# mcbuehler/DeepSEE

Measured on AMD Instinct MI355X. Metric: train-step images/sec (G+D fwd+bwd), 8x 32->256 bs=8, higher is better.
Workload: dtype fp32

## Files before the change

### deepsee_amd/csrc/elementwise.hip

```cpp
#include "dsee_common.h"
#include "dsee_rng.h"

namespace {

inline int egrid(long n) { return (int)min(8192L, (n + 255) / 256); }

__global__ __launch_bounds__(256) void up_noise_fwd_kernel(const float* __restrict__ x, const float* __restrict__ eps,
                                                           const float* __restrict__ nw, float* __restrict__ y, int N,
                                                           int H, int W, int C, int ups) {
  const long total4 = (long)N * H * W * C / 4;
  const int C4 = C / 4, h0 = H >> ups, w0 = W >> ups;
  for (long i = blockIdx.x * (long)blockDim.x + threadIdx.x; i < total4; i += (long)gridDim.x * blockDim.x) {
    const dsee_nhwq p = dsee_split_nhwq((unsigned)i, C4, W, H);
    const int q = p.q;
    f32x4 v = *reinterpret_cast<const f32x4*>(x + (((size_t)p.n * h0 + (p.h >> ups)) * w0 + (p.w >> ups)) * C + q * 4);
    if (eps) v += *reinterpret_cast<const f32x4*>(nw + q * 4) * *reinterpret_cast<const f32x4*>(eps + i * 4);
    *reinterpret_cast<f32x4*>(y + i * 4) = v;
  }
}

__global__ __launch_bounds__(256) void sumpool_kernel(const float* __restrict__ dy, float* __restrict__ dx, int N, int H,
                                                      int W, int C, int ups, float* __restrict__ amax = nullptr) {
  float vmax = 0.f;
  const int h0 = H >> ups, w0 = W >> ups, C4 = C / 4, f = 1 << ups;
// ... 368 lines not shown
                                                                uint64_t offset, const uint64_t* __restrict__ epoch) {
  if (epoch) offset += *epoch;
  __shared__ f32x4 red[256];
  const int tpp = C / 4, ppb = 256 / tpp > 0 ? 256 / tpp : 1;
  const int q = threadIdx.x % tpp, s = threadIdx.x / tpp;
  const bool active = threadIdx.x < ppb * tpp;
  const long p0 = (long)blockIdx.x * chunk_px, p1 = min(M, p0 + chunk_px);
  f32x4 acc = {0.f, 0.f, 0.f, 0.f};
  if (active)
    for (long p = p0 + s; p < p1; p += ppb)
      acc += *reinterpret_cast<const f32x4*>(a + p * C + q * 4) * philox_normal4(seed, offset + (uint64_t)(p * tpp + q));
  if (active) red[s * tpp + q] = acc;
  __syncthreads();
  if (active && s == 0) {
    f32x4 v = red[q];
    for (int j = 1; j < ppb; ++j) v += red[j * tpp + q];
    *reinterpret_cast<f32x4*>(part + (size_t)blockIdx.x * C + q * 4) = v;
  }
}

__global__ __launch_bounds__(256) void sumpool_dot_rng_kernel(const float* __restrict__ dy, float* __restrict__ dx, int N, int H,
                                                              int W, int C, int ups, float* __restrict__ amax,
                                                              float* __restrict__ part, uint64_t seed, uint64_t offset,
                                                              const uint64_t* __restrict__ epoch) {
  if (epoch) offset += *epoch;
  __shared__ f32x4 red[256];
  float vmax = 0.f;
  f32x4 acc = {0.f, 0.f, 0.f, 0.f};
  const int h0 = H >> ups, w0 = W >> ups, C4 = C / 4, f = 1 << ups;
  const long total4 = (long)N * h0 * w0 * C4;
  for (long i = blockIdx.x * (long)blockDim.x + threadIdx.x; i < total4; i += (long)gridDim.x * blockDim.x) {
    const dsee_nhwq p = dsee_split_nhwq((unsigned)i, C4, w0, h0);
    f32x4 v = {0.f, 0.f, 0.f, 0.f};
    for (int a = 0; a < f; ++a)
      for (int b = 0; b < f; ++b) {
        const size_t px = ((size_t)p.n * H + p.h * f + a) * W + p.w * f + b;
        const f32x4 d = *reinterpret_cast<const f32x4*>(dy + px * C + p.q * 4);
        v += d;
        acc += d * philox_normal4(seed, offset + (uint64_t)(px * C4 + p.q));
      }
    *reinterpret_cast<f32x4*>(dx + i * 4) = v;
    vmax = fmaxf(vmax, dsee_absmax4(v));
  }
  if (amax) dsee_block_atomic_absmax(amax, vmax);
  red[threadIdx.x] = acc;
  __syncthreads();
  if ((int)threadIdx.x < C4) {
    f32x4 s = red[threadIdx.x];
    for (int k = threadIdx.x + C4; k < 256; k += C4) s += red[k];
    *reinterpret_cast<f32x4*>(part + (size_t)blockIdx.x * C + threadIdx.x * 4) = s;
  }
}

}

extern "C" {

int dsee_upsample_noise_rng_fwd(const float* x, const float* noise_w, float* y, int N, int H, int W, int C, int ups,
                                uint64_t seed, uint64_t offset, hipStream_t st) {
  DSEE_CHECK_ARG(x && y && noise_w && C % 4 == 0);
  DSEE_CHECK_ARG((long)N * H * W * C / 4 < (1L << 32));
  up_noise_rng_fwd_kernel<false><<<egrid((long)N * H * W * C / 4), 256, 0, st>>>(x, noise_w, y, N, H, W, C, ups, seed, offset,
                                                                                 dsee_rng_epoch(), nullptr);
  DSEE_LAUNCH_CHECK();
  return DSEE_OK;
}

int dsee_upsample_noise_rng_fwd_stats(const float* x, const float* noise_w, float* y, int N, int H, int W, int C, int ups,
                                      uint64_t seed, uint64_t offset, float* stats_part, hipStream_t st) {
  DSEE_CHECK_ARG(x && y && noise_w && stats_part && C % 4 == 0 && C / 4 <= 256 && 256 % (C / 4) == 0);
  DSEE_CHECK_ARG((long)N * H * W * C / 4 < (1L << 32));
  const long items = (long)N * H * W * C / 4;
  const int grid = (int)min((long)DSEE_STATS_ROWS_MAX, (items + 255) / 256);
  up_noise_rng_fwd_kernel<true><<<grid, 256, 0, st>>>(x, noise_w, y, N, H, W, C, ups, seed, offset, dsee_rng_epoch(),
                                                      stats_part);
  DSEE_LAUNCH_CHECK();
  return DSEE_OK;
}

int dsee_channel_dot_rng(const float* a, float* out, long M, int C, float* workspace, uint64_t seed, uint64_t offset,
                         hipStream_t st) {
  DSEE_CHECK_ARG(a && out && workspace && C % 4 == 0 && C <= 1024);
  long cp = (M + 1023) / 1024;
  if (cp < 64) cp = 64;
  const int parts = (int)((M + cp - 1) / cp);
  chdot_rng_partial_kernel<<<parts, 256, 0, st>>>(a, workspace, M, C, (int)cp, seed, offset, dsee_rng_epoch());
  DSEE_LAUNCH_CHECK();
  chdot_finalize_kernel<<<C / 4, 256, 0, st>>>(workspace, parts, C, out);
  DSEE_LAUNCH_CHECK();
  return DSEE_OK;
}

int dsee_upsample_noise_fwd(const float* x, const float* eps, const float* noise_w, float* y, int N, int H, int W, int C,
                            int ups, hipStream_t st) {
  DSEE_CHECK_ARG(x && y && C % 4 == 0 && (eps == nullptr || noise_w != nullptr));
  DSEE_CHECK_ARG((long)N * H * W * C / 4 < (1L << 32));
  up_noise_fwd_kernel<<<egrid((long)N * H * W * C / 4), 256, 0, st>>>(x, eps, noise_w, y, N, H, W, C, ups);
  DSEE_LAUNCH_CHECK();
  return DSEE_OK;
}

int dsee_sumpool(const float* dy, float* dx, int N, int H, int W, int C, int ups, hipStream_t st) {
  DSEE_CHECK_ARG(dy && dx && C % 4 == 0 && ups >= 1);
  DSEE_CHECK_ARG((long)N * H * W * C / 4 < (1L << 32));
  sumpool_kernel<<<egrid((long)N * (H >> ups) * (W >> ups) * C / 4), 256, 0, st>>>(dy, dx, N, H, W, C, ups);
  DSEE_LAUNCH_CHECK();
  return DSEE_OK;
}

int dsee_sumpool_amax(const float* dy, float* dx, int N, int H, int W, int C, int ups, float* amax_dx, hipStream_t st) {
  DSEE_CHECK_ARG(dy && dx && amax_dx && C % 4 == 0 && ups >= 1);
  DSEE_CHECK_ARG((long)N * H * W * C / 4 < (1L << 32));
  sumpool_kernel<<<egrid((long)N * (H >> ups) * (W >> ups) * C / 4), 256, 0, st>>>(dy, dx, N, H, W, C, ups, amax_dx);
  DSEE_LAUNCH_CHECK();
  return DSEE_OK;
}

size_t dsee_sumpool_dot_rng_workspace(int N, int H, int W, int C, int ups) {
  return (size_t)egrid((long)N * (H >> ups) * (W >> ups) * C / 4) * C * sizeof(float);
}
int dsee_sumpool_dot_rng(const float* dy, float* dx, int N, int H, int W, int C, int ups, float* amax_dx, float* dnoise_w,
                         float* workspace, uint64_t seed, uint64_t offset, hipStream_t st) {
  DSEE_CHECK_ARG(dy && dx && dnoise_w && workspace && C % 4 == 0 && ups >= 1 && 256 % (C / 4) == 0);
  DSEE_CHECK_ARG((long)N * H * W * C / 4 < (1L << 32));
  const int grid = egrid((long)N * (H >> ups) * (W >> ups) * C / 4);
  sumpool_dot_rng_kernel<<<grid, 256, 0, st>>>(dy, dx, N, H, W, C, ups, amax_dx, workspace, seed, offset, dsee_rng_epoch());
  DSEE_LAUNCH_CHECK();
  chdot_finalize_kernel<<<C / 4, 256, 0, st>>>(workspace, grid, C, dnoise_w);
  DSEE_LAUNCH_CHECK();
  return DSEE_OK;
}

size_t dsee_channel_dot_workspace(long M, int C) {
  long cp = (M + 1023) / 1024;
  if (cp < 64) cp = 64;
  return (size_t)((M + cp - 1) / cp) * C * sizeof(float);
}

int dsee_channel_dot(const float* a, const float* b, float* out, long M, int C, float* workspace, hipStream_t st) {
  DSEE_CHECK_ARG(a && out && workspace && C % 4 == 0 && C <= 1024);
  long cp = (M + 1023) / 1024;
  if (cp < 64) cp = 64;
  const int parts = (int)((M + cp - 1) / cp);
  chdot_partial_kernel<<<parts, 256, 0, st>>>(a, b, workspace, M, C, (int)cp);
  DSEE_LAUNCH_CHECK();
  chdot_finalize_kernel<<<C / 4, 256, 0, st>>>(workspace, parts, C, out);
  DSEE_LAUNCH_CHECK();
  return DSEE_OK;
}

int dsee_act_fwd(const float* x, float* y, long n, int act, float slope, hipStream_t st) {
  DSEE_CHECK_ARG(x && y && n % 4 == 0);
  act_fwd_kernel<<<egrid(n / 4), 256, 0, st>>>(x, y, n / 4, act, slope);
  DSEE_LAUNCH_CHECK();
  return DSEE_OK;
}

int dsee_act_bwd(const float* dy, const float* y, float* dx, long n, int act, float slope, hipStream_t st) {
  DSEE_CHECK_ARG(dy && y && dx && n % 4 == 0);
  act_bwd_kernel<<<egrid(n / 4), 256, 0, st>>>(dy, y, dx, n / 4, act, slope);
  DSEE_LAUNCH_CHECK();
  return DSEE_OK;
}

int dsee_act_bwd_amax(const float* dy, const float* y, float* dx, long n, int act, float slope, float* amax_dx,
                      hipStream_t st) {
  DSEE_CHECK_ARG(dy && y && dx && amax_dx && n % 4 == 0);
  act_bwd_kernel<<<egrid(n / 4), 256, 0, st>>>(dy, y, dx, n / 4, act, slope, amax_dx);
  DSEE_LAUNCH_CHECK();
  return DSEE_OK;
}

int dsee_axpby(const float* a, float alpha, const float* b, float beta, float* y, long n, hipStream_t st) {
  DSEE_CHECK_ARG(a && y && n % 4 == 0);
  axpby_kernel<<<egrid(n / 4), 256, 0, st>>>(a, alpha, b, beta, y, n / 4);
  DSEE_LAUNCH_CHECK();
  return DSEE_OK;
}

int dsee_avgpool3s2_fwd(const float* x, float* y, int N, int H, int W, int C, hipStream_t st) {
  DSEE_CHECK_ARG(x && y && C % 4 == 0);
  const int Ho = (H + 2 - 3) / 2 + 1, Wo = (W + 2 - 3) / 2 + 1;
  avgpool3s2_fwd_kernel<<<egrid((long)N * Ho * Wo * C / 4), 256, 0, st>>>(x, y, N, H, W, Ho, Wo, C);
  DSEE_LAUNCH_CHECK();
  return DSEE_OK;
// ... 97 lines not shown
```

### deepsee_amd/networks.py

```python
import math
import re

import torch
import torch.nn as nn

from . import lib as L
from . import ops

NHIDDEN = ops.NHIDDEN


class Holder(nn.Module):
    """Pure container used to reproduce nn.Sequential-style key paths ('mlp_shared.0.weight')."""


def attach(root, dotted, module):
    parts = dotted.split(".")
    cur = root
    for p in parts[:-1]:
        if not hasattr(cur, p):
            cur.add_module(p, Holder())
        cur = getattr(cur, p)
    cur.add_module(parts[-1], module)
    return module
# ... 306 lines not shown
            actv = ops.SeanInput.apply(sh.weight, sh.bias, None, labels, shift, True, False)
        if self.kind == "spade":
            cat = ops.SeanInput.apply(sh.weight, sh.bias, None, labels, shift, True, False)
            w2, b2 = ops.pack_gamma_beta(self.mlp_gamma.weight, self.mlp_beta.weight, self.mlp_gamma.bias,
                                         self.mlp_beta.bias)
            add_one = 1.0
        elif self.kind == "sean":
            wg, wb = torch.sigmoid(self.alpha_gamma), torch.sigmoid(self.alpha_beta)
            if capped:
                wgam = (1.0 - wg) * self.mlp_gamma.weight + wg * self.mlp_style_gamma.weight
                wbet = (1.0 - wb) * self.mlp_beta.weight + wb * self.mlp_style_beta.weight
                cat = actv
            else:
                cat = ops.SeanInput.apply(sh.weight, sh.bias, style, labels, shift, True, True)
                wgam = torch.cat([(1.0 - wg) * self.mlp_gamma.weight, wg * self.mlp_style_gamma.weight], 1)
                wbet = torch.cat([(1.0 - wb) * self.mlp_beta.weight, wb * self.mlp_style_beta.weight], 1)
            bg = (1.0 - wg) * self.mlp_gamma.bias + wg * self.mlp_style_gamma.bias
            bb = (1.0 - wb) * self.mlp_beta.bias + wb * self.mlp_style_beta.bias
            w2, b2 = ops.pack_gamma_beta(wgam, wbet, bg, bb)
            add_one = 1.0
        else:
            cat = actv if capped else ops.SeanInput.apply(sh.weight, sh.bias, style, labels, shift, False, True)
            w2, b2 = ops.pack_gamma_beta(self.mlp_style_gamma.weight, self.mlp_style_beta.weight,
                                         self.mlp_style_gamma.bias, self.mlp_style_beta.bias)
            add_one = 0.0
        return ops.SpadeNormAct.apply(x, cat, w2, b2, *self._running(), training, add_one, cat_ups,
                                      grad_sink)


class SPADEResnetBlock(nn.Module):

    def __init__(self, c, opt, kind):
        super().__init__()
        self.kind, self.add_noise_cfg = kind, bool(opt.add_noise)
        self.conv_0 = SNConvP(c, c, 3, True)
        self.conv_1 = SNConvP(c, c, 3, True)
        norm = param_free_norm_of(opt.norm_G) if hasattr(opt, "norm_G") else "batch"
        self.norm_0 = SpadeNorm(kind, c, opt.semantic_nc, opt.regional_style_size, opt.max_fm_size, norm)
        self.norm_1 = SpadeNorm(kind, c, opt.semantic_nc, opt.regional_style_size, opt.max_fm_size, norm)
        if self.add_noise_cfg:
            self.noise_in, self.noise_skip, self.noise_middle = VecP(c), VecP(c), VecP(c)

    def forward(self, x, labels, style, noise, tag, ups, training, out_act=L.ACT_NONE, defer_act_bwd=False):
        noisy = self.add_noise_cfg and training
        n, h0, w0, c = x.shape
        shp = (n, h0 << ups, w0 << ups, c)
        res_noise = None
        if noisy:
            x = ops.UpNoise.apply(x, self.noise_in.weight, noise.normal_nhwc(shp, tag + ".noise_in"), ups, training)
            res_noise = (self.noise_skip.weight, noise.normal_nhwc(shp, tag + ".noise_skip"))
        elif ups:
            x = ops.UpNoise.apply(x, None, None, ups)
        sink = ops.GradSink() if (torch.is_grad_enabled() and x.requires_grad) else None
        h = self.norm_0(x, labels, style, training, sink)
        dx = ops.conv2d(h, self.conv_0.weight(training), self.conv_0.bias,
                        noise=(self.noise_middle.weight, noise.normal_nhwc(shp, tag + ".noise_middle")) if noisy else None,
                        stats=training)
        h = self.norm_1(dx, labels, style, training)
        return ops.conv2d(h, self.conv_1.weight(training), self.conv_1.bias, res=x, act=out_act, res_noise=res_noise,
                          res_sink=sink, defer_act_bwd=defer_act_bwd)


class DeepSEESR(nn.Module):

    def __init__(self, opt, plan):
        super().__init__()
        c = 16 * opt.ngf
        self.c = c
        self.initial = ConvP(c, 3, 3)
        self.head_0 = SPADEResnetBlock(c, opt, plan[0][1])
        self.G_middle_0 = SPADEResnetBlock(c, opt, plan[1][1])
        self.G_middle_1 = SPADEResnetBlock(c, opt, plan[2][1])
        self.up_list = nn.ModuleList([SPADEResnetBlock(c, opt, k) for _, k in plan[3:]])
        self.conv_img = ConvP(3, c, 3)
        self._sn = None

    def forward(self, image_lr, labels, style, noise, training):
        blocks = [("head_0", self.head_0, 0), ("G_middle_0", self.G_middle_0, 1), ("G_middle_1", self.G_middle_1, 0)]
        blocks += [("up_list.%d" % i, b, 1) for i, b in enumerate(self.up_list)]
        if self._sn is None:
            self._sn = ops.SNGroup([c for _, b, _ in blocks for c in (b.conv_0, b.conv_1)])
        self._sn.run(training)
        self._sn.wino_weights(torch.is_grad_enabled())
        x = ops.conv2d(image_lr, self.initial.weight, self.initial.bias)
        for i, (tag, blk, ups) in enumerate(blocks):
            last = i == len(blocks) - 1
            defer = last and torch.is_grad_enabled() and x.requires_grad and ops.P().defer_act
            x = blk(x, labels, style, noise, tag, ups, training, L.ACT_LRELU if last else L.ACT_NONE, defer)
        return ops.conv2d(x, self.conv_img.weight, self.conv_img.bias, act=L.ACT_TANH, in_act=L.ACT_LRELU if defer else 0)


class EncBranch(nn.Module):

    def __init__(self, names, strides, ups, nf, cin, norm="instance"):
        super().__init__()
        chans = [(nf, cin), (2 * nf, nf), (4 * nf, 2 * nf), (8 * nf, 4 * nf)]
        self.names, self.strides, self.ups = names, strides, ups
        self.norm_layers = [NormConv(self, nm, co, ci, 3, norm) for nm, (co, ci) in zip(names, chans)]

    def convs(self):
        return [nl.conv(self) for nl in self.norm_layers]

    def forward_main(self, x, training):
        for nl, s, u in zip(self.norm_layers, self.strides, self.ups):
            x = nl.apply(self, x, nl.conv(self).weight(training), L.ACT_LRELU, training, stride=s, pad=1, ups=u)
        return x
# ... 172 lines not shown
```

### deepsee_amd/ops.py

```python
import os
import ctypes as C

import threading

import torch

from . import lib as L
from .plan import KernelPlan, DEFAULT_PLAN, current as P

LRELU_SLOPE = 0.2
BN_EPS = 1e-5
BN_MOMENTUM = 0.1
SN_EPS = 1e-12
NHIDDEN = 128

_scratch = {}

PROFILE = None
PROFILE_BYTES = {}
PROFILE_OPERAND_GB = 0.0


def _variant(geom, modulate=False):
    halo = (geom.korder == 1 and geom.KH == 3 and geom.KW == 3 and geom.mul == 1 and geom.Hi == geom.Ho
# ... 803 lines not shown
            gd = L.geom_dgrad(geom)
            dxl = conv_raw(g, _pack_dgrad(w, geom.Cout, gd.korder), gd, amax_cache=getattr(ctx, "amax_cache", None),
                           exact=ctx.exact)
            if geom.ups:
                dx = torch.empty_like(x)
                L.call("sumpool", dxl, dx, geom.N, gd.Ho, gd.Wo, geom.Cin, geom.ups)
            else:
                dx = dxl
        if dw is not None or thin1:
            pass
        elif ctx.needs_input_grad[1] and ctx.thin:
            ws = scratch(L.lib().dsee_conv3x3_thin_wgrad_workspace(geom.Cin), "wgrad")
            dw = new(co, ci, 3, 3)
            L.call("conv3x3_thin_wgrad", x, g, ws, dw, geom.N, geom.Hi, geom.Wi, geom.Cin, co, ci)
        elif ctx.needs_input_grad[1] and ctx.wino and P().winograd_wgrad:
            dw = _wino_wgrad(x, g, geom.N, geom.Hi, geom.Wi, geom.Cin, geom.Cout, co, ci, vkeep, sums=sums)
        elif ctx.needs_input_grad[1]:
            dw = wgrad_raw(x, g, geom, co, ci, kh, kw, amax_cache=getattr(ctx, "amax_cache", None), exact=ctx.exact)
        if sums is not None and sums.get("dbias") is not None:
            db = sums["dbias"][:co]
        elif ctx.has_bias and ctx.needs_input_grad[2]:
            db = channel_dot(g, None, co).clone()
        if ctx.has_res and ctx.needs_input_grad[3]:
            if ctx.res_sink is not None:
                ctx.res_sink.put(g)
            else:
                dres = g

        def noise_wgrad(eps):
            cn = g.shape[-1]
            mrows = g.numel() // cn
            d = new(cn)
            L.call("channel_dot_rng", g, d, mrows, cn, scratch(L.lib().dsee_channel_dot_workspace(mrows, cn), "chdot"),
                   eps.seed, eps.offset)
            return d

        if sums is not None and "dn0" in sums:
            dnw, drnw = sums["dn0"], sums["dn1"]
        else:
            dnw = noise_wgrad(ctx.noise) if (ctx.noise is not None and ctx.needs_input_grad[8]) else None
            drnw = noise_wgrad(ctx.res_noise) if (ctx.res_noise is not None and ctx.needs_input_grad[10]) else None
        if ctx.in_act and dx is not None and not thin1:
            gx = torch.empty_like(dx)
            tag_amax(gx, amax_slot())
            L.call("act_bwd_amax", dx.contiguous(), x, gx, C.c_long(dx.numel()), ctx.in_act, LRELU_SLOPE, gx.dsee_amax)
            dx = gx
        return dx, dw, db, dres, None, None, None, None, dnw, None, drnw, None, None, None, None, None, None


class GradSink:

    def __init__(self):
        self.g = None

    def put(self, g):
        if self.g is not None:
            raise RuntimeError("GradSink holds a gradient nobody took: the previous backward pass did not reach the "
                               "normalisation that consumes it (partial backward passes are not supported)")
        self.g = g

    def take(self):
        g, self.g = self.g, None
        return g


def _fusable_noise(x, w, stride, pad, ups, eps):
    n, hi, wi, cin_s = x.shape
    return (P().fuse_noise and isinstance(eps, PhiloxNormal) and w.shape[2] == 3 and w.shape[0] > 4
            and _wino_ok(n, hi, wi, cin_s, L.pad4(w.shape[0]), 3, stride, pad, ups))


class ThinGather(torch.autograd.Function):
    @staticmethod
    def forward(ctx, z, bias, co, act, kh=3, kw=3, pad=1):
        n, h, w, ldz = z.shape
        ho, wo = h + 2 * pad - kh + 1, w + 2 * pad - kw + 1
        out = new(n, ho, wo, 4)
        if (kh, kw, pad) == (3, 3, 1):
            L.call("thin_gather_fwd", z, bias, out, n, h, w, ldz, co, act, LRELU_SLOPE)
        else:
            L.call("thin_gather_k_fwd", z, bias, out, n, h, w, ldz, co, kh, kw, pad, act, LRELU_SLOPE)
        ctx.save_for_backward(out)
        ctx.meta = (co, act, ldz, bias is not None, kh, kw, pad, h, w)
        return out

    @staticmethod
    def backward(ctx, dout):
        (out,) = ctx.saved_tensors
        co, act, ldz, has_bias, kh, kw, pad, h, w = ctx.meta
        n = out.shape[0]
        dout = dout.contiguous()
        dz = new(n, h, w, ldz)
        if (kh, kw, pad) == (3, 3, 1):
            L.call("thin_gather_bwd", dout, out, dz, n, h, w, ldz, co, act, LRELU_SLOPE)
        else:
            L.call("thin_gather_k_bwd", dout, out, dz, n, h, w, ldz, co, kh, kw, pad, act, LRELU_SLOPE)
        db = None
        if has_bias and ctx.needs_input_grad[1]:
            g = torch.empty_like(dout)
            L.call("act_bwd", dout, out, g, C.c_long(dout.numel()), act, LRELU_SLOPE)
            db = channel_dot(g, None, co).clone()
        return dz, db, None, None, None, None, None


def _thin_ok(x, w, res, stride, pad, ups, noise, res_noise):
    co, ci, kh, kw = w.shape
# ... 183 lines not shown
            L.call("counter_inc", counter)
        y = torch.empty_like(x)
        ao = amax_slot() if (_direct_split_on() and P().conv_amax_out) else None
        L.call("bn_act_fwd", x, mean, invstd, gamma, beta, y, n, h * w, c, act, LRELU_SLOPE, ao)
        if ao is not None:
            tag_amax(y, ao)
        ctx.act, ctx.emit_amax, ctx.cfg, ctx.training = act, ao is not None, cfg, training
        ctx.save_for_backward(x, y, mean, invstd, gamma)
        return y

    @staticmethod
    def backward(ctx, dy):
        assert ctx.training, "BatchNormAct: backward of an eval-mode forward"
        x, y, mean, invstd, gamma = ctx.saved_tensors
        n, h, w, c = x.shape
        dy = dy.contiguous()
        sums = new(2, c)
        ws = scratch(L.lib().dsee_norm_workspace(n, h * w, c, 1), "norm")
        L.call("bn_act_bwd_reduce", dy, y, x, mean, invstd, n, h * w, c, ctx.act, LRELU_SLOPE, sums, ws)
        count, local, cfg = n * h * w, None, ctx.cfg
        if cfg is not None:
            from . import parallel
            local = sums.clone()
            parallel.allreduce_sums(sums, cfg.world, cfg.group)
            count *= cfg.world
        dgamma = new(c) if ctx.needs_input_grad[1] else None
        dbeta = new(c) if ctx.needs_input_grad[2] else None
        dx = torch.empty_like(x)
        ao = amax_slot() if ctx.emit_amax else None
        L.call("bn_act_bwd_apply", dy, y, x, mean, invstd, gamma, sums, local, 1.0 / count, dx, dgamma, dbeta, n, h * w, c,
               ctx.act, LRELU_SLOPE, ao)
        if ao is not None:
            tag_amax(dx, ao)
        return dx, dgamma, dbeta, None, None, None, None, None


class Act(torch.autograd.Function):
    @staticmethod
    def forward(ctx, x, act):
        y = torch.empty_like(x)
        L.call("act_fwd", x, y, C.c_long(x.numel()), act, LRELU_SLOPE)
        ctx.act = act
        ctx.save_for_backward(y)
        return y

    @staticmethod
    def backward(ctx, dy):
        (y,) = ctx.saved_tensors
        dx = torch.empty_like(y)
        L.call("act_bwd", dy.contiguous(), y, dx, C.c_long(y.numel()), ctx.act, LRELU_SLOPE)
        return dx, None


class UpNoise(torch.autograd.Function):

    @staticmethod
    def forward(ctx, x, noise_w, eps, ups, stats=False):
        ctx.plan = P()
        n, h0, w0, c = x.shape
        y = new(n, h0 << ups, w0 << ups, c)
        ctx.philox = eps if isinstance(eps, PhiloxNormal) else None
        _bind_rng(eps)
        if ctx.philox is not None:
            assert eps.shape == tuple(y.shape)
            if stats and P().producer_stats and _stats_rows_ok(c):
                rows = L.lib().dsee_stats_part_rows(C.c_long(y.numel() // 4))
                part = new(rows, 3, c)
                L.call("upsample_noise_rng_fwd_stats", x, noise_w, y, n, h0 << ups, w0 << ups, c, ups, C.c_uint64(eps.seed),
                       C.c_uint64(eps.offset), part)
                y.dsee_stats_rows = (part, rows)
            else:
                L.call("upsample_noise_rng_fwd", x, noise_w, y, n, h0 << ups, w0 << ups, c, ups, C.c_uint64(eps.seed),
                       C.c_uint64(eps.offset))
            eps = None
        else:
            L.call("upsample_noise_fwd", x, eps, noise_w if eps is not None else None, y, n, h0 << ups, w0 << ups, c, ups)
        ctx.ups = ups
        ctx.save_for_backward(eps)
        ctx.xshape = x.shape
        return y

    @staticmethod
    @_under_plan
    def backward(ctx, dy):
        (eps,) = ctx.saved_tensors
        _bind_rng(ctx.philox)
        dy = dy.contiguous()
        n, h, w, c = dy.shape
        dx = dw = None
        if (ctx.ups and ctx.philox is not None and ctx.needs_input_grad[0] and ctx.needs_input_grad[1] and P().fuse_noise
                and 256 % (c // 4) == 0):
            dx, dw = new(*ctx.xshape), new(c)
            tag_amax(dx, amax_slot())
            ws = scratch(L.lib().dsee_sumpool_dot_rng_workspace(n, h, w, c, ctx.ups), "chdot")
            L.call("sumpool_dot_rng", dy, dx, n, h, w, c, ctx.ups, dx.dsee_amax, dw, ws, C.c_uint64(ctx.philox.seed),
                   C.c_uint64(ctx.philox.offset))
            return dx, dw, None, None, None
        if ctx.needs_input_grad[0]:
            if ctx.ups:
                dx = new(*ctx.xshape)
                tag_amax(dx, amax_slot())
                L.call("sumpool_amax", dy, dx, n, h, w, c, ctx.ups, dx.dsee_amax)
            else:
                dx = dy
        if ctx.philox is not None and ctx.needs_input_grad[1]:
            m = dy.numel() // c
            ws = scratch(L.lib().dsee_channel_dot_workspace(C.c_long(m), c), "chdot")
            dw = new(c)
            L.call("channel_dot_rng", dy, dw, C.c_long(m), c, ws, C.c_uint64(ctx.philox.seed),
                   C.c_uint64(ctx.philox.offset))
        elif eps is not None and ctx.needs_input_grad[1]:
            dw = channel_dot(dy, eps, c).clone()
        return dx, dw, None, None, None


class SeanInput(torch.autograd.Function):

    @staticmethod
    def forward(ctx, w_sh, b_sh, style, labels, shift, want_actv, want_style):
        n, h, w, nc = labels.n, labels.h, labels.w, labels.nc
        r, rw = h >> shift, w >> shift
        ld = (NHIDDEN if want_actv else 0) + (style.shape[2] if want_style else 0)
        cat = new(n, r, rw, ld)
        coff = 0
        if want_actv:
            table = new(9, nc, NHIDDEN)
            L.call("onehot_conv3x3_pack", w_sh.contiguous(), table, NHIDDEN, nc)
            L.call("onehot_conv3x3_fwd", labels.t, table, b_sh, cat, n, h, w, shift, nc, NHIDDEN, ld, 0, 1, -1, None, 0.0)
            coff = NHIDDEN
        if want_style:
            L.call("label_gather", labels.t, style.contiguous(), cat, n, h, w, shift, nc, style.shape[2], ld, coff, 1.0)
        ctx.labels, ctx.shift, ctx.want_actv, ctx.want_style, ctx.coff = labels, shift, want_actv, want_style, coff
        ctx.sshape = style.shape if want_style else None
        ctx.save_for_backward(cat)
        return cat

    @staticmethod
    def backward(ctx, dcat):
# ... 153 lines not shown
        if part is None:
            part = torch.empty(L.lib().dsee_norm_workspace(n, h * w, c, 1) // 4, dtype=torch.float32, device="cuda")
            L.call("norm_stats_partial", x, n, h * w, c, 1, part)
            if P().share_stats:
                x.dsee_stats_part = part
        L.call("norm_stats_finalize", part, n, h * w, c, 1, BN_EPS, BN_MOMENTUM, mean, invstd, running_mean, running_var)
        return mean, invstd, None
    ws = scratch(L.lib().dsee_norm_workspace(n, h * w, c, 1), "norm")
    from . import parallel
    local = new(2, c)
    L.call("norm_stats_local", x, n, h * w, c, local, ws)
    rows = parallel.gather_stats(local, cfg.world, cfg.group)
    L.call("norm_stats_merge", rows, cfg.world, n * h * w, c, BN_EPS, BN_MOMENTUM, int(cfg.clamp), mean, invstd,
           running_mean, running_var)
    return mean, invstd, cfg


def in_stats(x):
    n, h, w, c = x.shape
    mean, invstd = new(n, c), new(n, c)
    part = getattr(x, "dsee_in_part", None)
    if part is None:
        part = torch.empty(L.lib().dsee_norm_workspace(n, h * w, c, n) // 4, dtype=torch.float32, device="cuda")
        L.call("norm_stats_partial", x, n, h * w, c, n, part)
        if P().share_stats:
            x.dsee_in_part = part
    L.call("norm_stats_finalize", part, n, h * w, c, n, BN_EPS, BN_MOMENTUM, mean, invstd, None, None)
    return mean, invstd


def norm_stats(x, running_mean, running_var, training):
    if running_mean is None:
        mean, invstd = in_stats(x)
        return mean, invstd, None
    return bn_stats(x, running_mean, running_var, training)


def stat_groups(mean):
    return mean.shape[0] if mean.dim() == 2 else 1


def _call_sg(name, sg, head, tail):
    if sg == 1:
        L.call(name, *head, *tail)
    else:
        L.call(name + "_sg", *head, sg, *tail)


def _wino_ws(n, h, w, c, sg):
    return (L.lib().dsee_modulate_bwd_wino_workspace(n, h, w, c) if sg == 1
            else L.lib().dsee_modulate_bwd_wino_workspace_sg(n, h, w, c, sg))


def modulate_bwd(dh, out, x, scale, mean, invstd, rows, cfg, as_dm=False, add=None, xhat_amax=None, mask=None):
    n, h, w, c = x.shape
    sg = stat_groups(mean)
    dx = torch.empty_like(x)
    sums = new(2 * sg + 2, c)
    dgb = dm = None
    t = n * (h // 4) * (w // 4)
    dha = carried_amax(dh)
    pre = (as_dm and P().presplit_dm and P().presplit_gb and xhat_amax is not None and dha is not None and t % 256 == 0
           and sg == 1)
    s16 = scale.dtype == torch.float16
    if s16 and not (pre and P().half):
        scale, s16 = scale.float(), False
    if pre:
        ga = amax_slot()
        L.call("amax_product", dha, xhat_amax, 1.0, ga)
        pk = P().half
        dm = (_i16(36 * t * rows * (1 if pk else 2)), ga, "pk" if pk else True)
        ws = scratch(L.lib().dsee_modulate_bwd_wino_workspace(n, h, w, c), "norm")
        L.call("modulate_bwd_reduce_wino_f16p" if pk else "modulate_bwd_reduce_wino_f16x2", dh.contiguous(),
               None if mask is not None else out, x, scale, mean, invstd, dm[0], rows, sums, n, h, w, c, LRELU_SLOPE, ws, ga,
               DM_BOUND, mask)
    elif as_dm:
        dm = (new(36, t, rows), amax_slot() if (P().gemm_split and (P().gemm_f16x2 or P().half)) else None)
        ws = scratch(_wino_ws(n, h, w, c, sg), "norm")
        _call_sg("modulate_bwd_reduce_wino", sg, (dh.contiguous(), out, x, scale, mean, invstd, dm[0], rows, sums, n, h, w, c),
                 (LRELU_SLOPE, ws, dm[1]))
    else:
        dgb = (torch.zeros if c % 64 else torch.empty)(n, h, w, rows, dtype=torch.float32, device=x.device)
        ws = scratch(L.lib().dsee_norm_workspace(n, h * w, c, sg), "norm")
        _call_sg("modulate_bwd_reduce", sg, (dh.contiguous(), out, x, scale, mean, invstd, dgb, rows, sums, n, h * w, c),
                 (LRELU_SLOPE, ws))
    count = (n // sg) * h * w
    if cfg is not None:
        from . import parallel
        parallel.allreduce_sums(sums[0:2], cfg.world, cfg.group)
        count *= cfg.world
    da = amax_slot()
    _call_sg("modulate_bwd_apply_amax", sg,
             (dh.contiguous(), None if mask is not None else out, x, scale, mean, invstd, sums, add, dx, n, h * w, c),
             (1.0 / count, LRELU_SLOPE, da, int(s16), mask))
    tag_amax(dx, da)
    return dx, dgb, sums[2 * sg:2 * sg + 2], dm


class SpadeNormAct(torch.autograd.Function):

    @staticmethod
    def forward(ctx, x, cat, w2, b2, running_mean, running_var, training, add_one, cat_ups, grad_sink=None):
        ctx.plan = P()
        ctx.grad_sink = grad_sink
        n, h, w, c = x.shape
        rows, kin = w2.shape[0], w2.shape[1]
        assert cat.shape[3] == kin and kin % 4 == 0
        mean, invstd, ctx.sync = norm_stats(x, running_mean, running_var, training)
        geom = L.geom_fwd(n, cat.shape[1], cat.shape[2], kin, rows, 3, 1, 1, cat_ups)
        assert geom.Ho == h and geom.Wo == w
        w2 = w2.contiguous()
        out, scale = torch.empty_like(x), torch.empty_like(x)
        wp = _pack_fwd(w2, kin, geom.korder)
        with _timed(_variant(geom, True), _flops(geom)):
            _call_sg("conv2d_modulate_fwd", stat_groups(mean),
                     (C.byref(geom), cat, wp, None, 0, b2.contiguous(), x, mean, invstd, out, scale, c),
                     (float(add_one), LRELU_SLOPE))
        ctx.geom = geom
        ctx.save_for_backward(x, cat, w2, out, scale, mean, invstd)
        return out

    @staticmethod
    @_under_plan
    def backward(ctx, dh):
        x, cat, w2, out, scale, mean, invstd = ctx.saved_tensors
        geom = ctx.geom
        n, h, w, c = x.shape
        rows, kin = w2.shape[0], w2.shape[1]
        add = ctx.grad_sink.take() if ctx.grad_sink is not None else None
        dx, dgb, cs, _ = modulate_bwd(dh, out, x, scale, mean, invstd, rows, ctx.sync, add=add)
        dcat = dw2 = db2 = None
        if ctx.needs_input_grad[1]:
            gd = L.geom_dgrad(geom)
            dcl = conv_raw(dgb, _pack_dgrad(w2, rows, gd.korder), gd)
            if geom.ups:
                dcat = torch.empty_like(cat)
                L.call("sumpool", dcl, dcat, n, gd.Ho, gd.Wo, kin, geom.ups)
            else:
                dcat = dcl
        if ctx.needs_input_grad[2]:
            dw2 = wgrad_raw(cat, dgb, geom, rows, kin, 3, 3)
        if ctx.needs_input_grad[3]:
            idx, _ = packed_perm(c, x.device)
# ... 105 lines not shown
            kp = L.kpad(1, 1, ld)
            b2c = b2.contiguous()
            split = _split_kind(ld, rows)
            keep = [] if (P().keep_v and need_scale and nb == n and _wgrad_mode(ld, rows) == 2) else None
            for n0 in range(0, n, nb):
                if has_t:
                    ua = weight_amax(w2a if has_a else None, tb[n0:n0 + nb]) if split >= 2 else None
                    u = _i16(36 * nb * rows * kp * {1: 3, 2: 2, 3: 1}[split]) if split else new(36, nb, rows, kp)
                    L.call("wino43_weights_table", w2a if has_a else None, tb[n0:n0 + nb], u, nb, rows, ca, int(split),
                           ua)
                else:
                    u, ua = _wino_u(w2a, rows, ca, False, rows, kp, split)
                m, ms = _wino_vgemm(cat[n0:n0 + nb], nb, h, w, ld, u, rows, rows, kp, has_t, split, keep, ua)
                px = nb * h * w
                with _timed("spade_modulate_fused", 0.0,
                            (2.0 if split == 3 else 4.0) * 36 * (px // 16) * rows
                            + 4.0 * px * c * (3 if need_scale else 2)):
                    mc, ic = (mean, invstd) if sg == 1 else (mean[n0:n0 + nb], invstd[n0:n0 + nb])
                    _call_sg("wino43_output_modulate", 1 if sg == 1 else nb,
                             (m, b2c, x[n0:n0 + nb], mc, ic, out[n0:n0 + nb], scale[n0:n0 + nb] if need_scale else None, nb, h,
                              w, c, rows), (float(add_one), LRELU_SLOPE, ms))
        else:
            wp = _pack_fwd(w2a, ca, 1) if has_a else None
            with _timed(_variant(geom, True), _flops(geom)):
                _call_sg("conv2d_modulate_fwd", sg, (C.byref(geom), cat, wp, tb, ca, b2.contiguous(), x, mean, invstd, out,
                                                      scale, c), (float(add_one), LRELU_SLOPE))
        ctx.geom, ctx.labels, ctx.shift, ctx.has_a, ctx.has_t, ctx.rows = geom, labels, shift, has_a, has_t, rows
        ctx.cat_ups = cat_ups
        vcat = keep[0] if (nb and keep) else (None, None)
        ctx.v_kind = vcat[2] if len(vcat) == 3 else None
        ctx.w_amax = getattr(w2a, "dsee_amax", None) if has_a else None
        ctx.save_for_backward(x, cat, w2a if has_a else None, out, scale, mean, invstd, *vcat[:2], actv_low)
        return out

    @staticmethod
    @_under_plan
    def backward(ctx, dh):
        x, cat, w2a, out, scale, mean, invstd, vc, vc_amax, actv_low = ctx.saved_tensors
        if w2a is not None:
            w2a.dsee_amax = ctx.w_amax
        vcat = ((vc, vc_amax, ctx.v_kind) if ctx.v_kind else (vc, vc_amax)) if vc is not None else None
        geom, lab, shift, rows = ctx.geom, ctx.labels, ctx.shift, ctx.rows
        n, h, w, c = x.shape
        ld = cat.shape[3]
        dw_sh = db_sh = dw2a = dtable = db2 = None
        nb = ctx.wino_nb
        wino_w = bool(nb) and (ctx.has_t or ctx.needs_input_grad[3])
        fused_d = (wino_w and ctx.has_a and _wgrad_mode(ld, rows) != 1 and _adjoint_ok(rows, NHIDDEN))
        dactv_fused = [None]
        as_dm = (P().fuse_dm and wino_w and nb == n and _wgrad_mode(ld, rows) != 1 and (fused_d or not ctx.has_a)
                 and 256 % (c // 4) == 0)
        add = ctx.grad_sink.take() if ctx.grad_sink is not None else None
        pre_ok = vcat is not None and len(vcat) == 3 and _wgrad_mode(ld, rows) == 2 and (not ctx.has_a or fused_d)
        dx, dgb, cs, dm_all = modulate_bwd(dh, out, x, scale, mean, invstd, rows, ctx.sync, as_dm, add,
                                           getattr(ctx, "xhat_amax", None) if pre_ok else None,
                                           getattr(ctx, "sign_mask", None))

        def wino_wgrad():
            dw2a = dtable = None
            tpi, ca = (h // 4) * (w // 4), (NHIDDEN if ctx.has_a else 0)
            if fused_d:
                rows_t = L.wrows(NHIDDEN)
                u_t = _wino_u(w2a, rows, NHIDDEN, 2, rows_t, L.kpad(1, 1, rows),
                              4 if _is_pk(dm_all) else _split_kind(rows, NHIDDEN))
                dactv_fused[0] = new(n, h, w, NHIDDEN) if nb != n else None
            if ctx.has_t:
                nbytes = L.lib().dsee_wino43_wgrad_table_workspace(C.c_long(nb * tpi), nb, ca, rows)
                dtable = new(n, 9, rows, 32)
            else:
                nbytes = L.lib().dsee_wino43_wgrad_workspace(C.c_long(nb * tpi), ld, rows)
            wsw = scratch(nbytes, "wgrad")
            mode = _wgrad_mode(ld, rows)
            for n0 in range(0, n, nb):
                v, dm = _wino_wgrad_operands(cat[n0:n0 + nb], None if as_dm else dgb[n0:n0 + nb], nb, h, w, ld, rows,
                                             mode, vcat if (mode == 2 and nb == n) else None, dm_all)
                dwc = new(rows, NHIDDEN, 3, 3) if ctx.has_a else None
                with _timed(_wgrad_name(mode), 2.0 * 36 * nb * tpi * ld * rows):
                    if ctx.has_t:
                        L.call("wino43_wgrad_table", v[0], dm[0], wsw, nbytes, dwc, dtable[n0:n0 + nb], nb * tpi, nb, ca,
                               rows, lab.nc, _wgrad_code(v, dm, mode), v[1], dm[1])
                    else:
                        L.call("wino43_wgrad", v[0], dm[0], wsw, nbytes, dwc, nb * tpi, ld, rows, rows, NHIDDEN,
                               _wgrad_code(v, dm, mode), v[1], dm[1])
                if dwc is not None:
                    dw2a = dwc if dw2a is None else dw2a.add_(dwc)
                if fused_d:
                    dac = _wino_dgrad_from_dm(dm, u_t, nb, h, w, rows, NHIDDEN, rows_t,
                                              cat[n0:n0 + nb] if ctx.has_t else None, ld if ctx.has_t else 0)
                    if nb == n:
                        dactv_fused[0] = dac
                    else:
                        dactv_fused[0][n0:n0 + nb].copy_(dac)
            return dw2a, dtable

        if fused_d:
            dw2a, dtable = wino_wgrad()
        if ctx.has_a:
            ga = L.ConvGeom(n, h, w, rows, h, w, NHIDDEN, 3, 3, 1, 1, -1, 0, 0, 1)
            wino_d = ctx.wino_nb and _wino_chunk(n, h, w, rows) is not None
            if ctx.has_t:
                if fused_d:
                    dactv = dactv_fused[0]
                elif wino_d:
                    dactv = _wino_conv(dgb, w2a, n, h, w, NHIDDEN, rows, True, None, cat, L.ACT_MASK, res_ld=ld)
                else:
                    dactv = conv_raw(dgb, _pack_dgrad(w2a, rows, 1), ga, None, cat, L.ACT_MASK, res_ld=ld)
                gs = L.geom_fwd(n, h, w, ld, NHIDDEN, 3, 1, 1, 0)
                known = {}
                if getattr(ctx, "cat_amax", None) is not None:
# ... 170 lines not shown
```

### deepsee_amd/plan.py

```python
import contextlib
import dataclasses
import threading
from typing import Any, Optional


@dataclasses.dataclass(frozen=True)
class KernelPlan:
    winograd: bool = True
    winograd_wgrad: bool = True
    winograd_mod: bool = True
    gemm_split: bool = True
    gemm_af32: bool = True
    keep_v: bool = True
    gemm_f16x2: bool = True
    half: bool = False
    half_norms: bool = True
    presplit_a: bool = True
    gemm_w4: bool = True
    dgrad_s2_parity: bool = True
    presplit_min_tiles: int = 512
    conv_halo_f16: bool = True
    onehot_wgrad_mfma: bool = True
    conv_amax_out: bool = True
    presplit_dm: bool = True
    presplit_gb: bool = True
    dout_sums: bool = True
    adjoint_dgrad: bool = True
    fuse_noise: bool = True
    thin_gemm: bool = True
    share_stats: bool = True
    producer_stats: bool = True
    fuse_dm: bool = True
    fused_norm: bool = True
    fused_w4: bool = False
    sign_mask: bool = True
    defer_act: bool = True
    branch_streams: bool = False
    conv_f16x2_min_flop: float = 1e9
    sync_bn: Optional[Any] = None

    def replace(self, **changes):
        return dataclasses.replace(self, **changes)

    @contextlib.contextmanager
    def active(self):
        prev = getattr(_tls, "plan", None)
        _tls.plan = self
        try:
            yield self
        finally:
            _tls.plan = prev

    @classmethod
    def fields(cls):
        return [f.name for f in dataclasses.fields(cls)]


def _env_overrides():
    import ast
    import os
    text = os.environ.get("DSEE_PLAN", "").strip()
    if not text:
        return {}
    out = {}
    for item in text.split(","):
        k, _, v = item.partition("=")
        k = k.strip()
        if k not in KernelPlan.fields():
            raise ValueError("DSEE_PLAN: unknown KernelPlan field %r (fields: %s)" % (k, ", ".join(KernelPlan.fields())))
        out[k] = ast.literal_eval(v.strip())
    return out


DEFAULT_PLAN = KernelPlan(**_env_overrides())
_tls = threading.local()


def current():
    return getattr(_tls, "plan", None) or DEFAULT_PLAN


# ... 11 lines not shown
```

### include/deepsee_hip.h

```cpp
#ifndef DEEPSEE_HIP_H
#define DEEPSEE_HIP_H

#include <stddef.h>
#include <stdint.h>

#ifdef __cplusplus
extern "C" {
#endif

#ifndef __HIP_INCLUDE_HIP_HIP_RUNTIME_API_H__
typedef struct ihipStream_t* hipStream_t;
#endif

#define DSEE_OK 0
#define DSEE_EINVAL (-1)
#define DSEE_ELAUNCH (-2)
#define DSEE_EUNSUPPORTED (-3)

#define DSEE_ACT_NONE 0
#define DSEE_ACT_LRELU 1
#define DSEE_ACT_RELU 2
#define DSEE_ACT_TANH 3
#define DSEE_ACT_MASK 4

// ... 251 lines not shown
                                 const float* bias_packed, const float* x, const float* mean, const float* invstd,
                                 float* out_h, float* out_scale, int N, int H, int W, int C, int rows, int K, int groups,
                                 int stat_groups, float add_one, float slope, float* amax_h, float* amax_xhat,
                                 uint32_t* sign_mask, hipStream_t stream);
int dsee_wino43_output_modulate_sg(const float* M, const float* bias_packed, const float* x, const float* mean,
                                   const float* invstd, float* out_h, float* out_scale, int N, int H, int W, int C, int rows,
                                   int stat_groups, float add_one, float slope, const float* mscale, hipStream_t stream);
int dsee_conv2d_modulate_fwd_sg(const dsee_conv_geom* g, const float* in, const float* w_packed,
                                const float* style_table, int shared_cin, const float* bias_packed, const float* x,
                                const float* mean, const float* invstd, float* out_h, float* out_scale, int C,
                                int stat_groups, float add_one, float slope, hipStream_t stream);
int dsee_modulate_bwd_reduce_sg(const float* dh, const float* h, const float* x, const float* scale, const float* mean,
                                const float* invstd, float* dgb, int dgb_ld, float* sums, int N, int HW, int C,
                                int stat_groups, float slope, float* workspace, hipStream_t stream);
size_t dsee_modulate_bwd_wino_workspace_sg(int N, int H, int W, int C, int stat_groups);
int dsee_modulate_bwd_reduce_wino_sg(const float* dh, const float* h, const float* x, const float* scale,
                                     const float* mean, const float* invstd, float* dM, int rows, float* sums, int N, int H,
                                     int W, int C, int stat_groups, float slope, float* workspace, float* amax,
                                     hipStream_t stream);
int dsee_modulate_bwd_apply_amax_sg(const float* dh, const float* h, const float* x, const float* scale, const float* mean,
                                    const float* invstd, const float* sums, const float* add, float* dx, int N, int HW, int C,
                                    int stat_groups, float inv_count, float slope, float* amax_dx, int scale_f16,
                                    const uint32_t* sign_mask, hipStream_t stream);

int dsee_onehot_conv3x3_pack(const float* w_oihw, float* table, int Co, int L, hipStream_t stream);
int dsee_onehot_conv3x3_fwd(const uint8_t* lab, const float* table, const float* bias, float* out, int N, int H, int W,
                            int shift, int L, int Co, int out_ld, int coff, int relu, int onehot_coff, float* amax,
                            float amax_floor, hipStream_t stream);
size_t dsee_onehot_conv3x3_wgrad_workspace(int N, int H, int W, int shift, int L);
int dsee_onehot_conv3x3_wgrad(const uint8_t* lab, const float* dact, int dact_ld, const float* act, int act_ld, int N,
                              int H, int W, int shift, int L, float* dw_oihw, float* dbias, float* workspace,
                              hipStream_t stream);
int dsee_label_onehot(const uint8_t* lab, float* out, int N, int H, int W, int shift, int out_ld, int coff,
                      hipStream_t stream);
int dsee_label_gather(const uint8_t* lab, const float* table, float* out, int N, int H, int W, int shift, int L, int Cs,
                      int out_ld, int coff, float scale, hipStream_t stream);
size_t dsee_label_segsum_workspace(int N, int H, int W, int shift, int L, int Cs);
int dsee_label_segsum(const uint8_t* lab, const float* in, int ld, int coff, float* table, int N, int H, int W,
                      int shift, int L, int Cs, float scale, float* workspace, hipStream_t stream);

int dsee_upsample_noise_fwd(const float* x, const float* eps, const float* noise_w, float* y, int N, int H, int W, int C,
                            int ups, hipStream_t stream);
int dsee_upsample_noise_rng_fwd(const float* x, const float* noise_w, float* y, int N, int H, int W, int C, int ups,
                                uint64_t seed, uint64_t offset, hipStream_t stream);
int dsee_upsample_noise_rng_fwd_stats(const float* x, const float* noise_w, float* y, int N, int H, int W, int C, int ups,
                                      uint64_t seed, uint64_t offset, float* stats_part, hipStream_t stream);
int dsee_channel_dot_rng(const float* a, float* out, long M, int C, float* workspace, uint64_t seed, uint64_t offset,
                         hipStream_t stream);
int dsee_sumpool(const float* dy, float* dx, int N, int H, int W, int C, int ups, hipStream_t stream);
int dsee_sumpool_amax(const float* dy, float* dx, int N, int H, int W, int C, int ups, float* amax_dx, hipStream_t stream);
size_t dsee_sumpool_dot_rng_workspace(int N, int H, int W, int C, int ups);
int dsee_sumpool_dot_rng(const float* dy, float* dx, int N, int H, int W, int C, int ups, float* amax_dx, float* dnoise_w,
                         float* workspace, uint64_t seed, uint64_t offset, hipStream_t stream);
size_t dsee_channel_dot_workspace(long M, int C);
int dsee_channel_dot(const float* a, const float* b, float* out, long M, int C, float* workspace, hipStream_t stream);
int dsee_act_fwd(const float* x, float* y, long n, int act, float slope, hipStream_t stream);
int dsee_act_bwd(const float* dy, const float* y, float* dx, long n, int act, float slope, hipStream_t stream);
int dsee_act_bwd_amax(const float* dy, const float* y, float* dx, long n, int act, float slope, float* amax_dx,
                      hipStream_t stream);
int dsee_axpby(const float* a, float alpha, const float* b, float beta, float* y, long n, hipStream_t stream);
int dsee_avgpool3s2_fwd(const float* x, float* y, int N, int H, int W, int C, hipStream_t stream);
int dsee_avgpool3s2_bwd(const float* dy, float* dx, int N, int H, int W, int C, hipStream_t stream);
int dsee_maxpool2_fwd(const float* x, float* y, int N, int H, int W, int C, hipStream_t stream);
int dsee_maxpool2_bwd(const float* dy, const float* x, float* dx, int N, int H, int W, int C, hipStream_t stream);
int dsee_nchw_to_nhwc(const float* x, float* y, int N, int C, int H, int W, int Cs, hipStream_t stream);
int dsee_nhwc_to_nchw(const float* x, float* y, int N, int C, int H, int W, int Cs, hipStream_t stream);
int dsee_label_to_u8(const float* label, uint8_t* out, long n, hipStream_t stream);
int dsee_bicubic_down(const float* x, float* y, int N, int H, int W, int S, int cs_in, int cs_out, hipStream_t stream);
int dsee_image_u8_to_nhwc(const uint8_t* img, const uint8_t* flip, float* out, int N, int H, int W, int cs_out,
                          hipStream_t stream);
int dsee_label_u8_prepare(const uint8_t* lab, const uint8_t* flip, uint8_t* out, int N, int H, int W, int unknown_to,
                          hipStream_t stream);
int dsee_build_d_input(const uint8_t* lab, const float* img, float* out, long pixels, int L, int Cs, int img_cs,
                       hipStream_t stream);
int dsee_build_d_input_amax(const uint8_t* lab, const float* img, float* out, long pixels, int L, int Cs, int img_cs,
                            float* amax_out, hipStream_t stream);
int dsee_extract_image_grad(const float* din, float* dimg, long pixels, int L, int Cs, int img_cs, hipStream_t stream);
int dsee_rng_fill(float* out, long n, uint64_t seed, uint64_t offset, int normal, hipStream_t stream);
int dsee_rng_set_epoch(const uint64_t* epoch_dev);

size_t dsee_loss_workspace(void);
int dsee_loss_fwd_bwd(int mode, const float* a, const float* b, float* grad, long rows, int ld, int valid_c,
                      float weight, float* loss_out, float* workspace, hipStream_t stream);
int dsee_loss_bwd(int mode, const float* a, const float* b, float* grad, long rows, int ld, int valid_c, float weight,
                  const float* upstream, hipStream_t stream);

int dsee_sean_pack_rows(int C);
int dsee_sean_pack_fwd(const float* w_gamma, const float* w_beta, const float* ws_gamma, const float* ws_beta,
                       const float* b_gamma, const float* b_beta, const float* bs_gamma, const float* bs_beta,
                       const float* alpha_gamma, const float* alpha_beta, int mode, int C, int K, int S, float* w2a,
                       float* wst, float* b2, float* amax_w2a, hipStream_t stream);
size_t dsee_sean_pack_bwd_workspace(void);
int dsee_sean_pack_bwd(const float* w_gamma, const float* w_beta, const float* ws_gamma, const float* ws_beta,
                       const float* b_gamma, const float* b_beta, const float* bs_gamma, const float* bs_beta,
                       const float* alpha_gamma, const float* alpha_beta, int mode, int C, int K, int S,
                       const float* dw2a, const float* dwst, const float* db2, float* dw_gamma, float* dw_beta,
                       float* dws_gamma, float* dws_beta, float* db_gamma, float* db_beta, float* dbs_gamma,
                       float* dbs_beta, float* dalpha, float* workspace, hipStream_t stream);
int dsee_style_table_layout(const float* t, float* table, int N, int L, int rows, float* amax, hipStream_t stream);
int dsee_style_table_layout_bwd(const float* dtable, float* dt, int N, int L, int rows, hipStream_t stream);

int dsee_spectral_norm_fwd(const float* w_orig, float* u, float* v, float* sigma, float* w_sn, int R, int K,
                           int power_iter, float eps, float* scratch, hipStream_t stream);
int dsee_spectral_norm_bwd(const float* dw, const float* w_sn, const float* u, const float* v, const float* sigma,
                           float* dw_orig, int R, int K, float* scratch, hipStream_t stream);

// ... 108 lines not shown
```

Baseline: 93.50.

## Fuse SPADE norm backward apply with upsample-noise sumpool and noise-weight grad

Adds a kernel that computes the normalization backward apply (leaky-ReLU select, scale, mean/invstd correction, residual add) and then directly sum-pools the full-resolution gradient to the low-resolution input while accumulating the Philox noise dot product for the noise weight gradient. The autograd plumbing passes the UpNoise producer through the GradSink so the norm backward can produce the upsample gradient early, and UpNoise.backward just returns the stashed result. This avoids writing and re-reading the full-resolution dx tensor and one extra kernel launch per noisy block. The cost is more complex cross-op coupling and a dummy expanded dx being returned upstream, which relies on no other consumer needing the real full-resolution gradient.

```diff
diff --git a/deepsee_amd/csrc/elementwise.hip b/deepsee_amd/csrc/elementwise.hip
--- a/deepsee_amd/csrc/elementwise.hip
+++ b/deepsee_amd/csrc/elementwise.hip
@@ -444,6 +444,86 @@
   }
 }
 
+typedef _Float16 f16x4e __attribute__((ext_vector_type(4)));
+
+template <bool S16>
+__device__ __forceinline__ f32x4 norm_dx4(f32x4 dv, f32x4 sel, f32x4 xv, const float* __restrict__ scale, size_t e, f32x4 mu,
+                                          f32x4 is, f32x4 s0, f32x4 s1, float inv_count, const float* __restrict__ add) {
+#pragma clang fp contract(off)
+  f32x4 sc;
+  if constexpr (S16) {
+    const f16x4e h = *reinterpret_cast<const f16x4e*>(reinterpret_cast<const _Float16*>(scale) + e);
+    sc = (f32x4){(float)h[0], (float)h[1], (float)h[2], (float)h[3]};
+  } else {
+    sc = *reinterpret_cast<const f32x4*>(scale + e);
+  }
+  const f32x4 xh = (xv - mu) * is, g = dv * sel, a0 = s0 * inv_count, a1 = s1 * inv_count;
+  f32x4 r;
+#pragma unroll
+  for (int k = 0; k < 4; ++k) r[k] = is[k] * __builtin_fmaf(-a1[k], xh[k], __builtin_fmaf(g[k], sc[k], -a0[k]));
+  if (add) r = r + *reinterpret_cast<const f32x4*>(add + e);
+#pragma unroll
+  for (int k = 0; k < 4; ++k) asm volatile("" : "+v"(r[k]));
+  return r;
+}
+
+template <bool S16, int UPS>
+__global__ __launch_bounds__(256) void norm_bwd_apply_sumpool_rng_kernel(
+    const float* __restrict__ dh, const float* __restrict__ y, const float* __restrict__ x, const float* __restrict__ scale,
+    const float* __restrict__ mean, const float* __restrict__ invstd, const float* __restrict__ sums,
+    const float* __restrict__ add, float* __restrict__ dx, int N, int H, int W, int C, int ups, int groups, float inv_count,
+    float slope, const unsigned* __restrict__ mask, float* __restrict__ amax, float* __restrict__ part, uint64_t seed,
+    uint64_t offset, const uint64_t* __restrict__ epoch) {
+  if (epoch) offset += *epoch;
+  __shared__ f32x4 red[256];
+  float vmax = 0.f;
+  f32x4 acc = {0.f, 0.f, 0.f, 0.f};
+  if (UPS) ups = UPS;
+  constexpr int UNR = UPS ? 2 : 1;
+  const int h0 = H >> ups, w0 = W >> ups, C4 = C / 4, f = 1 << ups, ipg = N / groups;
+  const size_t npx = (size_t)N * H * W;
+  const long total4 = (long)N * h0 * w0 * C4;
+  for (long i = blockIdx.x * (long)blockDim.x + threadIdx.x; i < total4; i += (long)gridDim.x * blockDim.x) {
+    const dsee_nhwq p = dsee_split_nhwq((unsigned)i, C4, w0, h0);
+    const int c = p.q * 4;
+    const size_t sc = (size_t)(groups == 1 ? 0 : p.n / ipg) * C + c;
+    const f32x4 mu = *reinterpret_cast<const f32x4*>(mean + sc), is = *reinterpret_cast<const f32x4*>(invstd + sc);
+    const f32x4 s0 = *reinterpret_cast<const f32x4*>(sums + sc);
+    const f32x4 s1 = *reinterpret_cast<const f32x4*>(sums + (size_t)groups * C + sc);
+    f32x4 v = {0.f, 0.f, 0.f, 0.f};
+#pragma unroll UNR
+    for (int a = 0; a < f; ++a)
+#pragma unroll UNR
+      for (int b = 0; b < f; ++b) {
+        const size_t px = ((size_t)p.n * H + p.h * f + a) * W + p.w * f + b, e = px * C + c;
+        const f32x4 dv = *reinterpret_cast<const f32x4*>(dh + e);
+        f32x4 sel;
+        if (mask) {
+          const unsigned bits = mask[(size_t)(c >> 5) * npx + px] >> ((c & 31) >> 2);
+#pragma unroll
+          for (int k = 0; k < 4; ++k) sel[k] = (bits >> (8 * k)) & 1u ? 1.f : slope;
+        } else {
+          const f32x4 yv = *reinterpret_cast<const f32x4*>(y + e);
+#pragma unroll
+          for (int k = 0; k < 4; ++k) sel[k] = yv[k] > 0.f ? 1.f : slope;
+        }
+        const f32x4 d = norm_dx4<S16>(dv, sel, *reinterpret_cast<const f32x4*>(x + e), scale, e, mu, is, s0, s1, inv_count, add);
+        v += d;
+        acc += d * philox_normal4(seed, offset + (uint64_t)(px * C4 + p.q));
+      }
+    *reinterpret_cast<f32x4*>(dx + i * 4) = v;
+    vmax = fmaxf(vmax, dsee_absmax4(v));
+  }
+  if (amax) dsee_block_atomic_absmax(amax, vmax);
+  red[threadIdx.x] = acc;
+  __syncthreads();
+  if ((int)threadIdx.x < C4) {
+    f32x4 s = red[threadIdx.x];
+    for (int k = threadIdx.x + C4; k < 256; k += C4) s += red[k];
+    *reinterpret_cast<f32x4*>(part + (size_t)blockIdx.x * C + threadIdx.x * 4) = s;
+  }
+}
+
 }
 
 extern "C" {
@@ -523,6 +603,35 @@
   return DSEE_OK;
 }
 
+int dsee_norm_bwd_apply_sumpool_rng(const float* dh, const float* h, const float* x, const float* scale, const float* mean,
+                                    const float* invstd, const float* sums, const float* add, float* dx_low, int N, int H, int W,
+                                    int C, int stat_groups, int ups, float inv_count, float slope, int scale_f16,
+                                    const uint32_t* sign_mask, float* amax_dx, float* dnoise_w, float* workspace, uint64_t seed,
+                                    uint64_t offset, hipStream_t st) {
+  DSEE_CHECK_ARG(dh && (h || sign_mask) && x && scale && mean && invstd && sums && dx_low && dnoise_w && workspace);
+  DSEE_CHECK_ARG(C % 4 == 0 && 256 % (C / 4) == 0 && (!sign_mask || C % 32 == 0) && inv_count > 0.f);
+  DSEE_CHECK_ARG(ups >= 1 && ups < 16 && H % (1 << ups) == 0 && W % (1 << ups) == 0);
+  DSEE_CHECK_ARG(stat_groups == 1 || stat_groups == N);
+  DSEE_CHECK_ARG((long)N * H * W * C / 4 < (1L << 32));
+  const int grid = egrid((long)N * (H >> ups) * (W >> ups) * C / 4);
+#define DSEE_LAUNCH_FUSED(S16, UPS)                                                                                          \
+  norm_bwd_apply_sumpool_rng_kernel<S16, UPS><<<grid, 256, 0, st>>>(dh, h, x, scale, mean, invstd, sums, add, dx_low, N, H, W, C, \
+                                                                    ups, stat_groups, inv_count, slope, sign_mask, amax_dx,  \
+                                                                    workspace, seed, offset, dsee_rng_epoch())
+  if (scale_f16) {
+    if (ups == 1) DSEE_LAUNCH_FUSED(true, 1);
+    else DSEE_LAUNCH_FUSED(true, 0);
+  } else {
+    if (ups == 1) DSEE_LAUNCH_FUSED(false, 1);
+    else DSEE_LAUNCH_FUSED(false, 0);
+  }
+#undef DSEE_LAUNCH_FUSED
+  DSEE_LAUNCH_CHECK();
+  chdot_finalize_kernel<<<C / 4, 256, 0, st>>>(workspace, grid, C, dnoise_w);
+  DSEE_LAUNCH_CHECK();
+  return DSEE_OK;
+}
+
 size_t dsee_channel_dot_workspace(long M, int C) {
   long cp = (M + 1023) / 1024;
   if (cp < 64) cp = 64;
diff --git a/deepsee_amd/networks.py b/deepsee_amd/networks.py
--- a/deepsee_amd/networks.py
+++ b/deepsee_amd/networks.py
@@ -382,6 +382,8 @@
         elif ups:
             x = ops.UpNoise.apply(x, None, None, ups)
         sink = ops.GradSink() if (torch.is_grad_enabled() and x.requires_grad) else None
+        if sink is not None:
+            sink.producer = getattr(x, "dsee_upnoise", None)
         h = self.norm_0(x, labels, style, training, sink)
         dx = ops.conv2d(h, self.conv_0.weight(training), self.conv_0.bias,
                         noise=(self.noise_middle.weight, noise.normal_nhwc(shp, tag + ".noise_middle")) if noisy else None,
diff --git a/deepsee_amd/ops.py b/deepsee_amd/ops.py
--- a/deepsee_amd/ops.py
+++ b/deepsee_amd/ops.py
@@ -879,6 +879,7 @@
 
     def __init__(self):
         self.g = None
+        self.producer = None
 
     def put(self, g):
         if self.g is not None:
@@ -1168,6 +1169,17 @@
         return dx, None
 
 
+class UpNoiseGrad:
+
+    def __init__(self, philox, ups, xshape):
+        self.philox, self.ups, self.xshape = philox, ups, tuple(xshape)
+        self.result = None
+
+    def take(self):
+        r, self.result = self.result, None
+        return r
+
+
 class UpNoise(torch.autograd.Function):
 
     @staticmethod
@@ -1176,6 +1188,10 @@
         n, h0, w0, c = x.shape
         y = new(n, h0 << ups, w0 << ups, c)
         ctx.philox = eps if isinstance(eps, PhiloxNormal) else None
+        ctx.fused_grad = None
+        if (ups and ctx.philox is not None and ctx.needs_input_grad[0] and ctx.needs_input_grad[1] and P().fuse_noise
+                and P().fuse_norm_apply and 256 % (c // 4) == 0):
+            ctx.fused_grad = y.dsee_upnoise = UpNoiseGrad(ctx.philox, ups, x.shape)
         _bind_rng(eps)
         if ctx.philox is not None:
             assert eps.shape == tuple(y.shape)
@@ -1200,6 +1216,9 @@
     @_under_plan
     def backward(ctx, dy):
         (eps,) = ctx.saved_tensors
+        done = ctx.fused_grad.take() if ctx.fused_grad is not None else None
+        if done is not None:
+            return done[0], done[1], None, None, None
         _bind_rng(ctx.philox)
         dy = dy.contiguous()
         n, h, w, c = dy.shape
@@ -1459,10 +1478,9 @@
             else L.lib().dsee_modulate_bwd_wino_workspace_sg(n, h, w, c, sg))
 
 
-def modulate_bwd(dh, out, x, scale, mean, invstd, rows, cfg, as_dm=False, add=None, xhat_amax=None, mask=None):
+def modulate_bwd(dh, out, x, scale, mean, invstd, rows, cfg, as_dm=False, add=None, xhat_amax=None, mask=None, up=None):
     n, h, w, c = x.shape
     sg = stat_groups(mean)
-    dx = torch.empty_like(x)
     sums = new(2 * sg + 2, c)
     dgb = dm = None
     t = n * (h // 4) * (w // 4)
@@ -1496,6 +1514,17 @@
         from . import parallel
         parallel.allreduce_sums(sums[0:2], cfg.world, cfg.group)
         count *= cfg.world
+    if up is not None and P().fuse_norm_apply and (n, h >> up.ups, w >> up.ups, c) == up.xshape and 256 % (c // 4) == 0:
+        dxl, dnw = new(*up.xshape), new(c)
+        tag_amax(dxl, amax_slot())
+        ws = scratch(L.lib().dsee_sumpool_dot_rng_workspace(n, h, w, c, up.ups), "chdot")
+        _bind_rng(up.philox)
+        L.call("norm_bwd_apply_sumpool_rng", dh.contiguous(), None if mask is not None else out, x, scale, mean, invstd, sums,
+               add, dxl, n, h, w, c, sg, up.ups, 1.0 / count, LRELU_SLOPE, int(s16), mask, dxl.dsee_amax, dnw, ws,
+               C.c_uint64(up.philox.seed), C.c_uint64(up.philox.offset))
+        up.result = (dxl, dnw)
+        return x.new_empty(1).expand(x.shape), dgb, sums[2 * sg:2 * sg + 2], dm
+    dx = torch.empty_like(x)
     da = amax_slot()
     _call_sg("modulate_bwd_apply_amax", sg,
              (dh.contiguous(), None if mask is not None else out, x, scale, mean, invstd, sums, add, dx, n, h * w, c),
@@ -1707,9 +1736,10 @@
                  and 256 % (c // 4) == 0)
         add = ctx.grad_sink.take() if ctx.grad_sink is not None else None
         pre_ok = vcat is not None and len(vcat) == 3 and _wgrad_mode(ld, rows) == 2 and (not ctx.has_a or fused_d)
+        up = ctx.grad_sink.producer if (ctx.grad_sink is not None and add is not None) else None
         dx, dgb, cs, dm_all = modulate_bwd(dh, out, x, scale, mean, invstd, rows, ctx.sync, as_dm, add,
                                            getattr(ctx, "xhat_amax", None) if pre_ok else None,
-                                           getattr(ctx, "sign_mask", None))
+                                           getattr(ctx, "sign_mask", None), up)
 
         def wino_wgrad():
             dw2a = dtable = None
diff --git a/deepsee_amd/plan.py b/deepsee_amd/plan.py
--- a/deepsee_amd/plan.py
+++ b/deepsee_amd/plan.py
@@ -27,6 +27,7 @@
     dout_sums: bool = True
     adjoint_dgrad: bool = True
     fuse_noise: bool = True
+    fuse_norm_apply: bool = True
     thin_gemm: bool = True
     share_stats: bool = True
     producer_stats: bool = True
diff --git a/include/deepsee_hip.h b/include/deepsee_hip.h
--- a/include/deepsee_hip.h
+++ b/include/deepsee_hip.h
@@ -327,6 +327,11 @@
 size_t dsee_sumpool_dot_rng_workspace(int N, int H, int W, int C, int ups);
 int dsee_sumpool_dot_rng(const float* dy, float* dx, int N, int H, int W, int C, int ups, float* amax_dx, float* dnoise_w,
                          float* workspace, uint64_t seed, uint64_t offset, hipStream_t stream);
+int dsee_norm_bwd_apply_sumpool_rng(const float* dh, const float* h, const float* x, const float* scale, const float* mean,
+                                    const float* invstd, const float* sums, const float* add, float* dx_low, int N, int H, int W,
+                                    int C, int stat_groups, int ups, float inv_count, float slope, int scale_f16,
+                                    const uint32_t* sign_mask, float* amax_dx, float* dnoise_w, float* workspace, uint64_t seed,
+                                    uint64_t offset, hipStream_t stream);
 size_t dsee_channel_dot_workspace(long M, int C);
 int dsee_channel_dot(const float* a, const float* b, float* out, long M, int C, float* workspace, hipStream_t stream);
 int dsee_act_fwd(const float* x, float* y, long n, int act, float slope, hipStream_t stream);
```

Result: no change. 94.04, median of 6 (+0.6%).
